# facebookresearch/spdl

Hardware: AMD Instinct MI355X
Metric: images/sec device-resident JPEG→RGB224, 1/2/4/8×MI355X; % HBM roofline (higher is better)
Workload: dtype u8; 1 GPU; configs[1]: synthetic 480x640 q90 4:2:0 baseline JPEG resident in HBM -> RGB 224x224 u8 (scale bicubic decrease + centred pad, rgb24); global_batch=256, per_gpu_batch=256, distinct_images=32, lanes=4, hw_queues=4, entropy_threads=256, entropy_piece_bytes=131072

## Files before the change

spdl_amd/csrc/hj_kernels.hip:

```cpp
#include <hip/hip_fp16.h>
#include <hip/hip_runtime.h>

#include "hj_common.h"
#include "hj_destuff.h"
#include "hj_idct.h"

namespace hj {

__device__ __forceinline__ uint32_t rfl(uint32_t v) { return __builtin_amdgcn_readfirstlane(v); }


struct ParseScratch {
  ImageInfo info;
  uint16_t qt[4][64];
  uint8_t bits[8][17];
  uint8_t vals[8][256];
  int32_t have[8];
  int32_t qhave[4];
  int32_t maxcode[8][18];
  int32_t valoff[8][17];
  int32_t dqt_off[4], dqt_pq[4];
  int32_t dht_off[8], dht_n[8];
  int32_t qtsel[kMaxComp];
  int32_t comp_id[kMaxComp], comp_tq[kMaxComp], order[kMaxComp];
// ... 3787 lines not shown
        out[n++] = ((uint32_t)l[k] << 16) | (uint32_t)k;
      }
    }
    const int32_t dc = (int32_t)(int16_t)(uint16_t)((uint32_t)kDcBias + (uint32_t)l[0] * in.qt[c][0]);
    bdesc[(size_t)dd.coef_off + j] = make_uint2((uint32_t)j * 64u, n | ((uint32_t)dc << 16));
  }
  __syncthreads();
  if (tid == 0) {
    tph[3] = wall_clock64() - t0 - tph[0] - tph[1] - tph[2];
    for (int i = 0; i < 4; i++) in.tphase[i] = tph[i];
    for (int i = 0; i < 4; i++) in.dbg[i] = tdbg[i];
    for (int i = 0; i < 48; i++) in.sdiag[i] = S.sdiag[i];
    in.sync_rounds = S.nscans;
  }
}

hipError_t launch_multiscan(const uint8_t* bytes, uint8_t* clean, const ImageDesc* desc,
                            ImageInfo* infos, uint32_t* ents, uint2* bdesc, int n, hipStream_t st) {
  hipLaunchKernelGGL(multiscan_kernel, dim3(n), dim3(256), 0, st, bytes, clean, desc, infos, ents,
                     bdesc);
  return hipGetLastError();
}


constexpr int kBlkWords = 32;

typedef int16_t __attribute__((may_alias)) hj_i16_alias;

template <int NT>
__device__ __forceinline__ uint32_t slot_byte(uint32_t s) {
  return (s >> 1) * (uint32_t)NT * 4u + ((s & 1u) << 1);
}

template <int NT>
__device__ __forceinline__ void load_dequant(uint32_t (&sq)[kMaxComp][64], const ImageInfo& in,
                                             int tid) {
  for (int k = tid; k < kMaxComp * 64; k += NT)
    sq[k >> 6][k & 63] = slot_byte<NT>(kSlotOrder[k & 63]) | ((uint32_t)in.qt[k >> 6][k & 63] << 16);
}

template <int NT>
__device__ __forceinline__ void list_block(const uint32_t* __restrict__ ents, const uint2 bd,
                                           const int64_t coef_off, const int nblocks,
                                           const uint32_t* sqc, uint32_t* b32) {
#pragma unroll
  for (int w = 0; w < kBlkWords; w++) b32[w * NT] = w == 0 ? (bd.y >> 16) : 0u;
  uint8_t* blk = reinterpret_cast<uint8_t*>(b32);
  uint8_t* dummy = reinterpret_cast<uint8_t*>(b32 + kBlkWords * NT);
  const uint32_t cap = (uint32_t)nblocks * 64u;
  const uint32_t lo = bd.x & 3u, start = bd.x & ~3u;
  uint32_t count = min(bd.y & 0xFFFFu, 63u);
  if (start > cap - 64u) count = 0;
  const uint32_t hi_e = lo + count;
  const uint4* e4 = reinterpret_cast<const uint4*>(ents + (size_t)coef_off * 64 + start);
  const uint32_t n4 = (hi_e + 3u) >> 2;
  for (uint32_t i = 0; i < n4; i += 4) {
    uint4 q[4];
#pragma unroll
    for (int u = 0; u < 4; u++) q[u] = e4[min(i + u, n4 - 1u)];
#pragma unroll
    for (int u = 0; u < 4; u++) {
      const uint32_t w[4] = {q[u].x, q[u].y, q[u].z, q[u].w};
#pragma unroll
      for (int h = 0; h < 4; h++) {
        const uint32_t k = 4u * (i + u) + h;
        const uint32_t qs = sqc[w[h] & 63u];
        uint8_t* dst = k >= lo && k < hi_e ? blk + (qs & 0xFFFFu) : dummy;
        *reinterpret_cast<hj_i16_alias*>(dst) = (int16_t)pk_mul_lo16(w[h] >> 16, qs >> 16);
      }
    }
  }
}

typedef short hj_s16x2 __attribute__((ext_vector_type(2)));
__device__ __forceinline__ int32_t dot2(uint32_t a, uint32_t w, int32_t c) {
  return __builtin_amdgcn_sdot2(__builtin_bit_cast(hj_s16x2, a), __builtin_bit_cast(hj_s16x2, w),
                                c, false);
}
constexpr uint32_t pk16(int lo, int hi) {
  return (uint32_t)(uint16_t)(int16_t)lo | ((uint32_t)(uint16_t)(int16_t)hi << 16);
}
__device__ __forceinline__ uint32_t pack_lo16(uint32_t lo, uint32_t hi) {
  return __builtin_amdgcn_perm(hi, lo, 0x05040100u);
}
__device__ __forceinline__ void sidct8(uint32_t e0, uint32_t e1, uint32_t o0, uint32_t o1,
                                       int32_t bias, int32_t (&a)[4], int32_t (&b)[4]) {
  a[0] = dot2(e1, pk16(kW4, kW6), dot2(e0, pk16(kW4, kW2), bias));
  a[1] = dot2(e1, pk16(-kW4, -kW2), dot2(e0, pk16(kW4, kW6), bias));
  a[2] = dot2(e1, pk16(-kW4, kW2), dot2(e0, pk16(kW4, -kW6), bias));
  a[3] = dot2(e1, pk16(kW4, -kW6), dot2(e0, pk16(kW4, -kW2), bias));
  b[0] = dot2(o1, pk16(kW5, kW7), dot2(o0, pk16(kW1, kW3), 0));
  b[1] = dot2(o1, pk16(-kW1, -kW5), dot2(o0, pk16(kW3, -kW7), 0));
  b[2] = dot2(o1, pk16(kW7, kW3), dot2(o0, pk16(kW5, -kW1), 0));
  b[3] = dot2(o1, pk16(kW3, -kW1), dot2(o0, pk16(kW7, -kW5), 0));
}
template <int NT>
__device__ __forceinline__ uint4 blk_row(const uint32_t* b32, int i) {
  return make_uint4(b32[(4 * i) * NT], b32[(4 * i + 1) * NT], b32[(4 * i + 2) * NT],
                    b32[(4 * i + 3) * NT]);
}
template <int NT>
__device__ __forceinline__ void simple_idct_slots(const uint32_t* b32, int32_t (&px)[64]) {
  uint32_t r[8][8];
#pragma unroll
  for (int i = 0; i < 8; i++) {
    const uint4 q = blk_row<NT>(b32, i);
    int32_t a[4], b[4];
    sidct8(q.x, q.y, q.z, q.w, 1 << 10, a, b);
    const bool dc_only = ((q.x >> 16) | q.y | q.z | q.w) == 0u;
    const uint32_t dc = q.x << 3;
    r[i][0] = dc_only ? dc : (uint32_t)((int32_t)((uint32_t)a[0] + (uint32_t)b[0]) >> 11);
    r[i][7] = dc_only ? dc : (uint32_t)((int32_t)((uint32_t)a[0] - (uint32_t)b[0]) >> 11);
    r[i][1] = dc_only ? dc : (uint32_t)((int32_t)((uint32_t)a[1] + (uint32_t)b[1]) >> 11);
    r[i][6] = dc_only ? dc : (uint32_t)((int32_t)((uint32_t)a[1] - (uint32_t)b[1]) >> 11);
    r[i][2] = dc_only ? dc : (uint32_t)((int32_t)((uint32_t)a[2] + (uint32_t)b[2]) >> 11);
    r[i][5] = dc_only ? dc : (uint32_t)((int32_t)((uint32_t)a[2] - (uint32_t)b[2]) >> 11);
    r[i][3] = dc_only ? dc : (uint32_t)((int32_t)((uint32_t)a[3] + (uint32_t)b[3]) >> 11);
    r[i][4] = dc_only ? dc : (uint32_t)((int32_t)((uint32_t)a[3] - (uint32_t)b[3]) >> 11);
  }
#pragma unroll
  for (int k = 0; k < 8; k++) {
    int32_t a[4], b[4];
    sidct8(pack_lo16(r[0][k], r[2][k]), pack_lo16(r[4][k], r[6][k]), pack_lo16(r[1][k], r[3][k]),
           pack_lo16(r[5][k], r[7][k]), kW4 * ((1 << 19) / kW4), a, b);
    px[k] = clip_u8_opaque((int32_t)((uint32_t)a[0] + (uint32_t)b[0]) >> 20);
    px[8 + k] = clip_u8_opaque((int32_t)((uint32_t)a[1] + (uint32_t)b[1]) >> 20);
    px[16 + k] = clip_u8_opaque((int32_t)((uint32_t)a[2] + (uint32_t)b[2]) >> 20);
    px[24 + k] = clip_u8_opaque((int32_t)((uint32_t)a[3] + (uint32_t)b[3]) >> 20);
    px[32 + k] = clip_u8_opaque((int32_t)((uint32_t)a[3] - (uint32_t)b[3]) >> 20);
    px[40 + k] = clip_u8_opaque((int32_t)((uint32_t)a[2] - (uint32_t)b[2]) >> 20);
    px[48 + k] = clip_u8_opaque((int32_t)((uint32_t)a[1] - (uint32_t)b[1]) >> 20);
    px[56 + k] = clip_u8_opaque((int32_t)((uint32_t)a[0] - (uint32_t)b[0]) >> 20);
  }
}

template <int NT, int IDCT>
__device__ __forceinline__ void idct_block(const uint32_t* b32, int32_t (&px)[64]) {
  if (IDCT == 0) {
    simple_idct_slots<NT>(b32, px);
    return;
  }
  int32_t blk[64];
#pragma unroll
  for (int i = 0; i < 8; i++) {
    const uint4 q = blk_row<NT>(b32, i);
    blk[8 * i + 0] = sext16(q.x);
    blk[8 * i + 2] = sext16(q.x >> 16);
    blk[8 * i + 4] = sext16(q.y);
    blk[8 * i + 6] = sext16(q.y >> 16);
    blk[8 * i + 1] = sext16(q.z);
    blk[8 * i + 3] = sext16(q.z >> 16);
    blk[8 * i + 5] = sext16(q.w);
    blk[8 * i + 7] = sext16(q.w >> 16);
  }
  if (IDCT == 2) {
#pragma unroll
    for (int i = 0; i < 64; i++) px[i] = blk[i] & 255;
  } else {
    islow_block(blk, px);
  }
}

__device__ __forceinline__ void xcd_order(uint32_t& bx, uint32_t& by, uint32_t& bz) {
  const uint32_t n_wg = gridDim.x * gridDim.y * gridDim.z, full = n_wg & ~7u;
  uint32_t lin = bx + gridDim.x * (by + gridDim.y * bz);
  if (lin < full) lin = (lin & 7u) * (full >> 3) + (lin >> 3);
  bx = lin % gridDim.x;
  by = (lin / gridDim.x) % gridDim.y;
  bz = lin / (gridDim.x * gridDim.y);
}

template <int IDCT>
__global__ void __launch_bounds__(kIdctThreads) idct_kernel(const uint32_t* __restrict__ ents,
                                                            const uint2* __restrict__ bdesc,
                                                            const ImageDesc* __restrict__ desc,
                                                            const ImageInfo* __restrict__ infos,
                                                            uint8_t* __restrict__ planes,
                                                            const uint32_t* __restrict__ idct_map,
                                                            const int xcd) {
  __shared__ __attribute__((aligned(16))) uint32_t sblk[kBlkWords + 1][kIdctThreads];
  __shared__ uint32_t sq[kMaxComp][64];
  uint32_t gx = blockIdx.x, gy = blockIdx.y, gz = blockIdx.z;
  if (xcd) xcd_order(gx, gy, gz);
  const bool flat = idct_map != nullptr;
  const int img = flat ? (int)idct_map[gx] : (int)gy;
  const int tile = flat ? (int)gx - desc[img].idct_wg0 : (int)gx;
  const int j = tile * kIdctThreads + threadIdx.x;
  const ImageInfo& in = infos[img];
  if (in.status != kOk || tile * kIdctThreads >= in.nblocks) return;
  load_dequant<kIdctThreads>(sq, in, threadIdx.x);
  __syncthreads();
  if (j >= in.nblocks) return;
  const ImageDesc& dd = desc[img];
  const int bpm = in.bpm;
  const int mcu = j / bpm, b = j - mcu * bpm;
  const int c = in.mcu_comp[b];
  const int mx = mcu % in.mcux, my = mcu / in.mcux;
  int bx, by;
  if (in.ncomp == 1) {
    bx = mx;
    by = my;
  } else {
    bx = mx * in.comp_h[c] + in.mcu_dx[b];
    by = my * in.comp_v[c] + in.mcu_dy[b];
  }
  uint32_t* b32 = &sblk[0][threadIdx.x];
  list_block<kIdctThreads>(ents, bdesc[(size_t)dd.coef_off + j], dd.coef_off, in.nblocks, sq[c],
                           b32);
  int32_t px[64];
  idct_block<kIdctThreads, IDCT>(b32, px);
  const int stride = dd.plane_stride[c];
  uint8_t* dst = planes + dd.plane_off[c] + (size_t)by * 8 * stride + bx * 8;
#pragma unroll
  for (int r = 0; r < 8; r++) {
    uint2 v;
    v.x = (uint32_t)px[8 * r] | ((uint32_t)px[8 * r + 1] << 8) | ((uint32_t)px[8 * r + 2] << 16) |
          ((uint32_t)px[8 * r + 3] << 24);
    v.y = (uint32_t)px[8 * r + 4] | ((uint32_t)px[8 * r + 5] << 8) |
          ((uint32_t)px[8 * r + 6] << 16) | ((uint32_t)px[8 * r + 7] << 24);
    *reinterpret_cast<uint2*>(dst + (size_t)r * stride) = v;
  }
}


constexpr int32_t kFix1402 = 91881, kFix1772 = 116130, kFix0714 = 46802, kFix0344 = 22553;

__device__ __forceinline__ void ycc_rgb(int y, int cb, int cr, int* rgb) {
  const int32_t x_cb = cb - 128, x_cr = cr - 128;
  const int32_t cr_r = (kFix1402 * x_cr + 32768) >> 16;
  const int32_t cb_b = (kFix1772 * x_cb + 32768) >> 16;
  const int32_t g = ((-kFix0344 * x_cb + 32768) + (-kFix0714 * x_cr)) >> 16;
  rgb[0] = clip_u8(y + cr_r);
  rgb[1] = clip_u8(y + g);
  rgb[2] = clip_u8(y + cb_b);
}

__device__ __forceinline__ uint16_t to_f16_bits(float f, int dtype) {
  if (dtype == 1) return __half_as_ushort(__float2half_rn(f));
  uint32_t x = __float_as_uint(f);
  if ((x & 0x7FFFFFFFu) > 0x7F800000u) return (uint16_t)((x >> 16) | 0x40u);
  x += 0x7FFFu + ((x >> 16) & 1u);
  return (uint16_t)(x >> 16);
}

__device__ __forceinline__ void store_rgb(void* out, int64_t base, int fmt, int dtype, int ow,
                                          int oh, int x, int y, const int* rgb,
                                          const BatchParams& p) {
  const bool planar = fmt == 0 || fmt == 1;
  const bool swap = fmt == 1 || fmt == 3;
  const int64_t pl = (int64_t)ow * oh;
#pragma unroll
  for (int ch = 0; ch < 3; ch++) {
    const int v = rgb[swap ? 2 - ch : ch];
    const int64_t oi = base + (planar ? ch * pl + (int64_t)y * ow + x : ((int64_t)y * ow + x) * 3 + ch);
    if (dtype == 0) {
      static_cast<uint8_t*>(out)[oi] = (uint8_t)v;
    } else {
      float f = __fdiv_rn((float)v, 255.0f);
      f = __fsub_rn(f, p.mean[ch]);
      f = __fdiv_rn(f, p.std[ch]);
      static_cast<uint16_t*>(out)[oi] = to_f16_bits(f, dtype);
    }
  }
}

__global__ void __launch_bounds__(256) csc_kernel(const uint8_t* __restrict__ planes,
                                                  const ImageDesc* __restrict__ desc,
                                                  const ImageInfo* __restrict__ infos,
                                                  void* __restrict__ out, const BatchParams p,
                                                  int32_t* __restrict__ host_status) {
  const int img = blockIdx.y;
  const ImageInfo& in = infos[img];
  if (host_status && blockIdx.x == 0 && threadIdx.x == 0) host_status[img] = in.status;
  if (in.status != kOk) return;
  const ImageDesc& dd = desc[img];
  const int W = in.width, H = in.height;
  const int64_t npx = (int64_t)W * H;
  for (int64_t i = (int64_t)blockIdx.x * blockDim.x + threadIdx.x; i < npx;
       i += (int64_t)gridDim.x * blockDim.x) {
    const int y = (int)(i / W), x = (int)(i - (int64_t)y * W);
    const int lx = x * in.comp_h[0] / in.hmax, ly = y * in.comp_v[0] / in.vmax;
    const int yv = planes[dd.plane_off[0] + (int64_t)ly * dd.plane_stride[0] + lx];
    int rgb[3];
    if (in.ncomp == 1) {
      rgb[0] = rgb[1] = rgb[2] = yv;
    } else {
      const int cx1 = x * in.comp_h[1] / in.hmax, cy1 = y * in.comp_v[1] / in.vmax;
      const int cx2 = x * in.comp_h[2] / in.hmax, cy2 = y * in.comp_v[2] / in.vmax;
      const int cb = planes[dd.plane_off[1] + (int64_t)cy1 * dd.plane_stride[1] + cx1];
      const int cr = planes[dd.plane_off[2] + (int64_t)cy2 * dd.plane_stride[2] + cx2];
      if (in.color == kColorRgb) {
        rgb[0] = yv;
        rgb[1] = cb;
        rgb[2] = cr;
      } else {
        ycc_rgb(yv, cb, cr, rgb);
      }
    }
    store_rgb(out, dd.out_off, p.pix_fmt, p.dtype, W, H, x, y, rgb, p);
  }
}


typedef short hj_short2 __attribute__((ext_vector_type(2)));
typedef uint32_t hj_u32x4a __attribute__((ext_vector_type(4), aligned(4)));

template <int NW>
__device__ __forceinline__ void load_words(const uint8_t* p, uint32_t (&w)[NW]) {
  static_assert(NW % 4 == 0, "whole 16-byte loads");
#pragma unroll
  for (int i = 0; i < NW; i += 4) {
    const hj_u32x4a v = *reinterpret_cast<const hj_u32x4a*>(p + 4 * i);
    w[i] = v.x;
    w[i + 1] = v.y;
    w[i + 2] = v.z;
    w[i + 3] = v.w;
  }
}

template <int NQ, int NW>
__device__ __forceinline__ int32_t hdot(const uint32_t (&w)[NW], uint32_t sh, const uint32_t* wp) {
  int32_t h = 0;
#pragma unroll
  for (int i = 0; i < NQ; i++) {
    const uint32_t u = __builtin_amdgcn_alignbyte(w[i + 1], w[i], sh);
    const uint32_t lo = __builtin_amdgcn_perm(0u, u, 0x0C010C00u);
    const uint32_t hi = __builtin_amdgcn_perm(0u, u, 0x0C030C02u);
    h = __builtin_amdgcn_sdot2(__builtin_bit_cast(hj_short2, lo),
                               __builtin_bit_cast(hj_short2, wp[2 * i]), h, false);
    h = __builtin_amdgcn_sdot2(__builtin_bit_cast(hj_short2, hi),
                               __builtin_bit_cast(hj_short2, wp[2 * i + 1]), h, false);
  }
  return h;
}

__device__ __forceinline__ int16_t h15(int32_t h) {
  return (int16_t)min(h >> 7, (1 << 15) - 1);
}

template <int NQ>
__device__ __forceinline__ void hpass_cols(const uint8_t* plane, int stride, int ph, const int32_t* pos,
                           const int16_t* coef, int cstride, int c0, int ncols, int r0, int r1,
                           int16_t* lds, int cst, int tid, int nthreads, int rst = 1) {
  constexpr int NW = (NQ + 1 + 3) / 4 * 4;
  for (int c = tid; c < ncols; c += nthreads) {
    const int x = c0 + c;
    const int p = pos[x];
    const uint32_t sh = (uint32_t)(p & 3);
    uint32_t wp[2 * NQ];
    const uint2* cp = reinterpret_cast<const uint2*>(coef + (int64_t)x * cstride);
#pragma unroll
    for (int k = 0; k < NQ; k++) {
      const uint2 t = cp[k];
      wp[2 * k] = t.x;
      wp[2 * k + 1] = t.y;
    }
    const uint8_t* base = plane + (p & ~3);
    int16_t* out = lds + c * cst;
    constexpr int G = NW <= 4 ? 12 : (NW <= 8 ? 4 : 1);
    for (int r = r0; r < r1; r += G) {
      uint32_t w[G][NW];
#pragma unroll
      for (int g = 0; g < G; g++)
        if (r + g < r1) load_words<NW>(base + (int64_t)min(r + g, ph - 1) * stride, w[g]);
#pragma unroll
      for (int g = 0; g < G; g++)
        if (r + g < r1) out[(r + g - r0) * rst] = h15(hdot<NQ>(w[g], sh, wp));
    }
  }
}

__device__ __forceinline__ void hpass_cols_long(const uint8_t* plane, int stride, int ph, const int32_t* pos,
                                const int16_t* coef, int cstride, int taps, int c0, int ncols,
                                int r0, int r1, int16_t* lds, int cst, int tid, int nthreads,
                                int rst = 1) {
  for (int c = tid; c < ncols; c += nthreads) {
    const int x = c0 + c;
    const int p = pos[x];
    const int16_t* cf = coef + (int64_t)x * cstride;
    for (int r = r0; r < r1; r++) {
      const uint8_t* row = plane + (int64_t)min(r, ph - 1) * stride + p;
      int32_t v = 0;
      for (int t = 0; t < taps; t++) v += (int32_t)row[t] * cf[t];
      lds[c * cst + (r - r0) * rst] = h15(v);
    }
  }
}

__device__ __forceinline__ void hpass(const uint8_t* plane, int stride, int ph, const int32_t* pos,
                      const int16_t* coef, int cstride, int taps, int c0, int ncols, int r0, int r1,
                      int16_t* lds, int cst, int tid, int nthreads, int rst = 1) {
  const int nq = (taps + 3) >> 2;
#define HJ_HP(N) \
  hpass_cols<N>(plane, stride, ph, pos, coef, cstride, c0, ncols, r0, r1, lds, cst, tid, nthreads, \
                rst)
  if (nq <= 1) HJ_HP(1);
  else if (nq <= 2) HJ_HP(2);
  else if (nq <= 3) HJ_HP(3);
  else if (nq <= 4) HJ_HP(4);
  else if (nq <= 6) HJ_HP(6);
  else if (nq <= 8) HJ_HP(8);
  else if (nq <= 12) HJ_HP(12);
  else if (nq <= 16) HJ_HP(16);
  else hpass_cols_long(plane, stride, ph, pos, coef, cstride, taps, c0, ncols, r0, r1, lds, cst, tid,
                       nthreads, rst);
#undef HJ_HP
}

__device__ __forceinline__ int32_t vdot_pairs(const uint32_t* col, int p, const uint32_t* f,
                                              int np) {
  const uint32_t* c = col + (p >> 1);
  const uint32_t sh = (uint32_t)(p & 1) * 16u;
  int32_t acc = 0;
  uint32_t w0 = c[0];
  for (int i = 0; i < np; i += 2) {
    const uint32_t w1 = c[i + 1], w2 = c[i + 2];
    const uint2 ff = *reinterpret_cast<const uint2*>(f + i);
    acc = __builtin_amdgcn_sdot2(__builtin_bit_cast(hj_short2, __builtin_amdgcn_alignbit(w1, w0, sh)),
                                 __builtin_bit_cast(hj_short2, ff.x), acc, false);
    acc = __builtin_amdgcn_sdot2(__builtin_bit_cast(hj_short2, __builtin_amdgcn_alignbit(w2, w1, sh)),
                                 __builtin_bit_cast(hj_short2, ff.y), acc, false);
    w0 = w2;
  }
  return acc;
}

__device__ __forceinline__ void vpair(const uint32_t* col, int p, int& a, int& b) {
  const uint32_t* c = col + (p >> 1);
  const uint32_t w = __builtin_amdgcn_alignbit(c[1], c[0], (uint32_t)(p & 1) * 16u);
  a = (int32_t)(int16_t)(w & 0xFFFFu);
  b = (int32_t)w >> 16;
}

__device__ __forceinline__ int clip_i8(int v) { return v < 0 ? 0 : (v > 255 ? 255 : v); }

__device__ __forceinline__ int tab_off(int32_t inc, int c) {
  return ((clip_i8(c) * inc) >> 16) - (inc >> 9);
}

__device__ __forceinline__ void full_rgb(const BatchParams& p, int Y, int U, int V, int* rgb) {
  Y -= p.y_offset;
  Y *= p.y_coeff;
  Y += 1 << 21;
  int R = (int)((uint32_t)Y + (uint32_t)V * (uint32_t)p.v2r);
  int G = (int)((uint32_t)Y + (uint32_t)V * (uint32_t)p.v2g + (uint32_t)U * (uint32_t)p.u2g);
  int B = (int)((uint32_t)Y + (uint32_t)U * (uint32_t)p.u2b);
  if ((R | G | B) & 0xC0000000) {
    auto c30 = [](int a) { return (a & ~((1 << 30) - 1)) ? ((~a) >> 31) & ((1 << 30) - 1) : a; };
    R = c30(R);
    G = c30(G);
    B = c30(B);
  }
  rgb[0] = R >> 22;
  rgb[1] = G >> 22;
  rgb[2] = B >> 22;
}

__global__ void __launch_bounds__(256) hscale_kernel(const uint8_t* __restrict__ planes,
                                                     const ImageDesc* __restrict__ desc,
                                                     const ImageInfo* __restrict__ infos,
                                                     const int32_t* __restrict__ pool,
                                                     const uint32_t* __restrict__ hs_map,
                                                     int16_t* __restrict__ hbuf) {
  const int img = (int)hs_map[blockIdx.x];
  const ImageInfo& in = infos[img];
  if (in.status != kOk) return;
  const ImageDesc& dd = desc[img];
  const SwsDesc& s = dd.sws;
  const int32_t* T = pool + dd.wt_off;
  const int tl = (s.pre_rl + kHsRows - 1) / kHsRows;
  const int tc = s.gbr ? tl : (s.gray ? 0 : (s.pre_rc + kHsRows - 1) / kHsRows);
  int t = (int)blockIdx.x - dd.hs_wg0;
  int c = 0;
  if (t >= tl) {
    t -= tl;
    c = 1 + t / tc;
    t %= tc;
  }
  const bool lumaf = c == 0 || s.gbr;
  const int rows = lumaf ? s.pre_rl : s.pre_rc;
  const int w = lumaf ? s.sw : s.chr_w;
  const int r0 = t * kHsRows, r1 = min(r0 + kHsRows, rows);
  const int64_t pbase = c == 0 ? 0 : (int64_t)s.pre_rl * s.sw + (c == 1 ? 0 : (int64_t)rows * w);
  const uint8_t* plane = planes + dd.plane_off[c];
  const int stride = dd.plane_stride[c], ph = in.comp_hpx[c];
  const int32_t* pos = T + s.off[lumaf ? kHlPos : kHcPos];
  const int16_t* coef = reinterpret_cast<const int16_t*>(T + s.off[lumaf ? kHlCoef : kHcCoef]);
  const int cstride = lumaf ? s.hl_size : s.hc_size, taps = lumaf ? s.hl_taps : s.hc_taps;
  int16_t* dst = hbuf + dd.hbuf_off + pbase + (int64_t)r0 * w;
  if (taps <= 64) {
    hpass(plane, stride, ph, pos, coef, cstride, taps, 0, w, r0, r1, dst, 1, threadIdx.x,
          blockDim.x, w);
    return;
  }
  const int nch = (taps + 63) / 64;
  for (int x = threadIdx.x; x < w; x += blockDim.x) {
    const int p0 = pos[x];
    const uint32_t sh = (uint32_t)(p0 & 3);
    const uint8_t* base = plane + (p0 & ~3);
    int32_t acc[kHsRows];
#pragma unroll
    for (int g = 0; g < kHsRows; g++) acc[g] = 0;
    for (int k = 0; k < nch; k++) {
      uint32_t wp[32];
      const uint2* cp = reinterpret_cast<const uint2*>(coef + (int64_t)x * cstride + 64 * k);
#pragma unroll
      for (int q = 0; q < 16; q++) {
        const bool in_row = 64 * k + 4 * q < taps;
        const uint2 t = in_row ? cp[q] : make_uint2(0u, 0u);
        wp[2 * q] = t.x;
        wp[2 * q + 1] = t.y;
      }
#pragma unroll
      for (int g = 0; g < kHsRows; g++) {
        if (r0 + g >= r1) break;
        uint32_t wv[20];
        load_words<20>(base + (int64_t)min(r0 + g, ph - 1) * stride + 64 * k, wv);
        acc[g] += hdot<16>(wv, sh, wp);
      }
    }
#pragma unroll
    for (int g = 0; g < kHsRows; g++)
      if (r0 + g < r1) dst[(int64_t)g * w + x] = h15(acc[g]);
  }
}

__global__ void __launch_bounds__(256) sws_kernel(const uint8_t* __restrict__ planes,
                                                  const ImageDesc* __restrict__ desc,
                                                  const ImageInfo* __restrict__ infos,
                                                  const int32_t* __restrict__ pool,
                                                  void* __restrict__ out, const BatchParams p,
                                                  int32_t* __restrict__ host_status,
                                                  const int16_t* __restrict__ hbuf,
                                                  const uint32_t* __restrict__ sws_map) {
  extern __shared__ __attribute__((aligned(16))) int16_t sws_lds[];
  const bool flat = sws_map != nullptr;
  uint32_t bx = blockIdx.x, by = blockIdx.y, bz = blockIdx.z;
  if (p.xcd_order & 1) xcd_order(bx, by, bz);
  const int img = flat ? (int)sws_map[bx] : (int)bz, tid = threadIdx.x, nt = blockDim.x;
  const ImageDesc& dd = desc[img];
  const int t = flat ? (int)bx - dd.sws_wg0 : (int)(bx * dd.sws_chunks + by);
  const int band = flat ? t / dd.sws_chunks : (int)bx;
  const int chunk = flat ? t - band * dd.sws_chunks : (int)by;
  const ImageInfo& in = infos[img];
  if (host_status && t == 0 && tid == 0) host_status[img] = in.status;
  if (in.status != kOk) return;
  const SwsDesc& s = dd.sws;
  const int yo0 = band * s.rb, xo0 = chunk * s.col_chunk;
  if (yo0 >= dd.oh || xo0 >= dd.ow) return;
  const int yo1 = min(yo0 + s.rb, dd.oh), xo1 = min(xo0 + s.col_chunk, dd.ow);
  const int th = yo1 - yo0, tw = xo1 - xo0;
  const int ys0 = max(yo0 - dd.dy, 0), ys1 = min(yo1 - dd.dy, s.sh);
  const int xs0 = max(xo0 - dd.dx, 0), xs1 = min(xo1 - dd.dx, s.sw);
  const bool content = ys0 < ys1 && xs0 < xs1;
  const bool planar = p.pix_fmt == 0 || p.pix_fmt == 1;
  const bool swap = p.pix_fmt == 1 || p.pix_fmt == 3;
  const bool u8 = p.dtype == 0;
  const int64_t pl = (int64_t)dd.ow * dd.oh;
  const int32_t* T = pool + dd.wt_off;
  const int32_t* vl_pos = T + s.off[kVlPos];
  const int32_t* vc_pos = T + s.off[kVcPos];
  int lr0 = 0, lr1 = 0, cr0 = 0, cr1 = 0, cx0 = 0, ncc = 0;
  const int ncl = content ? xs1 - xs0 : 0;
  if (content) {
    lr0 = vl_pos[ys0];
    lr1 = vl_pos[ys1 - 1] + s.vl_taps;
    if (!s.gray) {
      cr0 = vc_pos[ys0];
      cr1 = vc_pos[ys1 - 1] + s.vc_taps;
      cx0 = s.full ? xs0 : xs0 >> 1;
      ncc = (s.full ? xs1 - 1 : (xs1 - 1) >> 1) + 1 - cx0;
    }
  }
  const int lst = sws_col_stride(lr1 - lr0), cst = sws_col_stride(cr1 - cr0);
  int16_t* hl = sws_lds;
  int16_t* hu = hl + ncl * lst;
  int16_t* hv = hu + (s.gbr ? ncl * lst : s.gray ? 0 : ncc * cst);
  const int hrow_end = (int)((hv + (s.gbr ? ncl * lst : s.gray ? 0 : ncc * cst)) - sws_lds);
  uint8_t* tile = reinterpret_cast<uint8_t*>(sws_lds) + ((2 * hrow_end + 15) & ~15);
  const int vrw = 4 + (s.vl_size + s.vc_size) / 2;
  uint32_t* vt = reinterpret_cast<uint32_t*>(tile + ((s.rb * s.col_chunk * 3 + 15) & ~15));
  if (content) {
    const int32_t* vmode = T + s.off[kVmode];
    const uint32_t* vlw = reinterpret_cast<const uint32_t*>(T + s.off[kVlCoef]);
    const uint32_t* vcw = reinterpret_cast<const uint32_t*>(T + s.off[kVcCoef]);
    const int nl = s.vl_size / 2, nc = s.vc_size / 2;
    for (int i = tid; i < (ys1 - ys0) * vrw; i += nt) {
      const int r = i / vrw, w = i - r * vrw, ys = ys0 + r;
      uint32_t v = 0;
      if (w == 0) v = (uint32_t)vmode[ys];
      else if (w == 1) v = (uint32_t)(vl_pos[ys] - lr0);
      else if (w == 2) v = s.gray ? 0u : (uint32_t)(vc_pos[ys] - cr0);
      else if (w >= 4 && w < 4 + nl) v = vlw[(int64_t)ys * nl + (w - 4)];
      else if (w >= 4 + nl) v = vcw[(int64_t)ys * nc + (w - 4 - nl)];
      vt[i] = v;
    }
  }
  auto put = [&](int xo, int yo, const int* rgb) {
    const int c0v = swap ? rgb[2] : rgb[0], c2v = swap ? rgb[0] : rgb[2];
    const int cv[3] = {c0v, rgb[1], c2v};
    if (u8) {
#pragma unroll
      for (int ch = 0; ch < 3; ch++) {
        const int v = cv[ch];
        const int ti = planar ? (ch * th + (yo - yo0)) * tw + (xo - xo0)
                              : ((yo - yo0) * tw + (xo - xo0)) * 3 + ch;
        tile[ti] = (uint8_t)v;
      }
      return;
    }
#pragma unroll
    for (int ch = 0; ch < 3; ch++) {
      const int v = cv[ch];
      const int64_t oi =
          dd.out_off + (planar ? ch * pl + (int64_t)yo * dd.ow + xo : ((int64_t)yo * dd.ow + xo) * 3 + ch);
      float f = __fdiv_rn((float)v, 255.0f);
      f = __fsub_rn(f, p.mean[ch]);
      f = __fdiv_rn(f, p.std[ch]);
      static_cast<uint16_t*>(out)[oi] = to_f16_bits(f, p.dtype);
    }
  };
  {
    const int npx = th * tw;
    const int zero[3] = {0, 0, 0};
    for (int i = tid; i < npx; i += nt) {
      const int yo = yo0 + i / tw, xo = xo0 + i % tw;
      const int ys = yo - dd.dy, xs = xo - dd.dx;
      if (ys < 0 || ys >= s.sh || xs < 0 || xs >= s.sw) put(xo, yo, zero);
    }
  }
  if (content && s.pre) {
    const int16_t* hb = hbuf + dd.hbuf_off;
    const int wl = s.sw, wc = s.gbr ? s.sw : s.chr_w;
    const int64_t cbase = (int64_t)s.pre_rl * wl;
    auto stage = [&](const int16_t* src, int w, int rows, int c0, int ncols, int r0, int r1,
                     int16_t* dst, int cst_) {
      const int nr = r1 - r0, ne = ncols * nr;
      for (int i0 = tid; i0 < ne; i0 += 4 * nt) {
        int16_t v[4];
#pragma unroll
        for (int u = 0; u < 4; u++) {
          const int i = min(i0 + u * nt, ne - 1);
          const int r = i / ncols, c = i - r * ncols;
          v[u] = src[(int64_t)min(r0 + r, rows - 1) * w + c0 + c];
        }
#pragma unroll
        for (int u = 0; u < 4; u++) {
          const int i = i0 + u * nt;
          if (i < ne) {
            const int r = i / ncols, c = i - r * ncols;
            dst[c * cst_ + r] = v[u];
          }
        }
      }
    };
    stage(hb, wl, s.pre_rl, xs0, ncl, lr0, lr1, hl, lst);
    if (s.gbr) {
      stage(hb + cbase, wl, s.pre_rl, xs0, ncl, lr0, lr1, hu, lst);
      stage(hb + 2 * cbase, wl, s.pre_rl, xs0, ncl, lr0, lr1, hv, lst);
    } else if (!s.gray) {
      const int64_t cpl = (int64_t)s.pre_rc * wc;
      stage(hb + cbase, wc, s.pre_rc, cx0, ncc, cr0, cr1, hu, cst);
      stage(hb + cbase + cpl, wc, s.pre_rc, cx0, ncc, cr0, cr1, hv, cst);
    }
  } else if (content && s.gbr) {
    const int third = nt / 3, c = min(tid / third, 2), t3 = tid - c * third;
    if (tid < 3 * third)
      hpass(planes + dd.plane_off[c], dd.plane_stride[c], in.comp_hpx[c], T + s.off[kHlPos],
            reinterpret_cast<const int16_t*>(T + s.off[kHlCoef]), s.hl_size, s.hl_taps, xs0, ncl,
            lr0, lr1, c == 0 ? hl : c == 1 ? hu : hv, lst, t3, third);
  } else if (content && !(p.debug_mask & 0x100)) {
    hpass(planes + dd.plane_off[0], dd.plane_stride[0], in.comp_hpx[0], T + s.off[kHlPos],
          reinterpret_cast<const int16_t*>(T + s.off[kHlCoef]), s.hl_size, s.hl_taps, xs0, ncl,
          lr0, lr1, hl, lst, tid, nt);
    if (!s.gray) {
      const int half = nt >> 1, t2 = tid < half ? tid : tid - half;
      const int c = tid < half ? 1 : 2;
      hpass(planes + dd.plane_off[c], dd.plane_stride[c], in.comp_hpx[c], T + s.off[kHcPos],
            reinterpret_cast<const int16_t*>(T + s.off[kHcCoef]), s.hc_size, s.hc_taps, cx0, ncc,
            cr0, cr1, c == 1 ? hu : hv, cst, t2, half);
    }
  }
  __syncthreads();
  if (content && !(p.debug_mask & 0x200)) {
    const int npl = s.vl_size / 2, npc = s.vc_size / 2;
    for (int cl = tid; cl < ncl; cl += nt) {
      const int xs = xs0 + cl;
      const int cc = (s.full ? xs : xs >> 1) - cx0;
      const uint32_t* lcol = reinterpret_cast<const uint32_t*>(hl + cl * lst);
      const uint32_t* ucol = reinterpret_cast<const uint32_t*>(hu + cc * cst);
      const uint32_t* vcol = reinterpret_cast<const uint32_t*>(hv + cc * cst);
      for (int ys = ys0; ys < ys1; ys++) {
        const uint32_t* row = vt + (ys - ys0) * vrw;
        const uint4 hdr = *reinterpret_cast<const uint4*>(row);
        const int m = (int)hdr.x;
        const int mode = m & 15, ya = (m >> 4) & 8191, ua = (m >> 17) & 8191;
        const uint32_t* lf = row + 4;
        const uint32_t* cf = lf + npl;
        const int lp = (int)hdr.y, cp = (int)hdr.z;
        int rgb[3];
        int Y, U = 0, V = 0;
        if (s.gbr) {
          const uint32_t* cols[3] = {lcol, lcol + (hu - hl) / 2, lcol + (hv - hl) / 2};
#pragma unroll
          for (int c = 0; c < 3; c++) {
            int v;
            if (mode == kSwsX) {
              v = ((1 << 18) + vdot_pairs(cols[c], lp, lf, npl)) >> 19;
            } else {
              int a, b;
              vpair(cols[c], lp, a, b);
              v = mode == kSwsTwo ? (a * (4096 - ya) + b * ya) >> 19 : (a + 64) >> 7;
            }
            rgb[c] = clip_i8(v);
          }
        } else if (s.full) {
          if (mode == kSwsTwo) {
            int a, b;
            vpair(lcol, lp, a, b);
            Y = (a * (4096 - ya) + b * ya) >> 10;
          } else if (mode == kSwsOne) {
            int a, b;
            vpair(lcol, lp, a, b);
            Y = a * 4;
          } else {
            Y = ((1 << 9) + vdot_pairs(lcol, lp, lf, npl)) >> 10;
          }
          if (!s.gray) {
            if (mode == kSwsX) {
              U = ((1 << 9) - (128 << 19) + vdot_pairs(ucol, cp, cf, npc)) >> 10;
              V = ((1 << 9) - (128 << 19) + vdot_pairs(vcol, cp, cf, npc)) >> 10;
            } else {
              int u0, u1, v0, v1;
              vpair(ucol, cp, u0, u1);
              vpair(vcol, cp, v0, v1);
              if (!ua) {
                u1 = u0;
                v1 = v0;
              }
              U = (u0 * (4096 - ua) + u1 * ua - (128 << 19)) >> 10;
              V = (v0 * (4096 - ua) + v1 * ua - (128 << 19)) >> 10;
            }
          }
          full_rgb(p, Y, U, V, rgb);
        } else {
          if (mode == kSwsX) {
            Y = ((1 << 18) + vdot_pairs(lcol, lp, lf, npl)) >> 19;
            U = ((1 << 18) + vdot_pairs(ucol, cp, cf, npc)) >> 19;
            V = ((1 << 18) + vdot_pairs(vcol, cp, cf, npc)) >> 19;
          } else {
            int y0, y1, u0, u1, v0, v1;
            vpair(lcol, lp, y0, y1);
            vpair(ucol, cp, u0, u1);
            vpair(vcol, cp, v0, v1);
            if (mode == kSwsTwo) {
              Y = (y0 * (4096 - ya) + y1 * ya) >> 19;
              U = (u0 * (4096 - ua) + u1 * ua) >> 19;
              V = (v0 * (4096 - ua) + v1 * ua) >> 19;
            } else {
              if (!ua) {
                u1 = u0;
                v1 = v0;
              }
              Y = (y0 + 64) >> 7;
              U = (u0 * (4096 - ua) + u1 * ua + (128 << 11)) >> 19;
              V = (v0 * (4096 - ua) + v1 * ua + (128 << 11)) >> 19;
            }
          }
          rgb[0] = clip_i8(Y + tab_off(p.crv, V));
          rgb[1] = clip_i8(Y + tab_off(p.cgu, U) + tab_off(p.cgv, V));
          rgb[2] = clip_i8(Y + tab_off(p.cbu, U));
        }
        put(xs + dd.dx, ys + dd.dy, rgb);
      }
    }
  }
  if (!u8 || (p.debug_mask & 0x400)) return;
  __syncthreads();
  const int nplane = planar ? 3 : 1;
  const int run = planar ? th * tw : th * tw * 3;
  for (int pc = 0; pc < nplane; pc++) {
    const uint8_t* src = tile + pc * run;
    uint8_t* dst = static_cast<uint8_t*>(out) + dd.out_off + pc * pl +
                   (planar ? (int64_t)yo0 * dd.ow + xo0 : ((int64_t)yo0 * dd.ow + xo0) * 3);
    if (tw == dd.ow && ((uintptr_t)dst & 15) == 0 && (run & 15) == 0) {
      for (int i = tid; i < run / 16; i += nt)
        reinterpret_cast<uint4*>(dst)[i] = reinterpret_cast<const uint4*>(src)[i];
    } else {
      const int rowb = planar ? tw : tw * 3;
      const int64_t ostride = planar ? dd.ow : (int64_t)dd.ow * 3;
      for (int i = tid; i < run; i += nt) {
        const int r = i / rowb, k = i - r * rowb;
        dst[r * ostride + k] = src[i];
      }
    }
  }
}

__device__ __forceinline__ void yuv_stage(const int16_t* __restrict__ src, int w, int rows, int c0,
                                          int ncols, int r0, int r1, int16_t* dst, int cst,
                                          int tid, int nt) {
  const int nr = r1 - r0, ne = ncols * nr;
  for (int i0 = tid; i0 < ne; i0 += 4 * nt) {
    int16_t v[4];
#pragma unroll
    for (int u = 0; u < 4; u++) {
      const int i = min(i0 + u * nt, ne - 1);
      const int r = i / ncols, c = i - r * ncols;
      v[u] = src[(int64_t)min(r0 + r, rows - 1) * w + c0 + c];
    }
#pragma unroll
    for (int u = 0; u < 4; u++) {
      const int i = i0 + u * nt;
      if (i < ne) {
        const int r = i / ncols, c = i - r * ncols;
        dst[c * cst + r] = v[u];
      }
    }
  }
}

__global__ void __launch_bounds__(256) yuv_planes_kernel(const uint8_t* __restrict__ planes,
                                                         const ImageDesc* __restrict__ desc,
                                                         const ImageInfo* __restrict__ infos,
                                                         const int32_t* __restrict__ pool,
                                                         uint8_t* __restrict__ out,
                                                         int32_t* __restrict__ host_status,
                                                         const int16_t* __restrict__ hbuf,
                                                         const uint32_t* __restrict__ sws_map) {
  extern __shared__ __attribute__((aligned(16))) int16_t yuv_lds[];
  const int img = (int)sws_map[blockIdx.x], tid = threadIdx.x, nt = blockDim.x;
  const ImageDesc& dd = desc[img];
  int t = (int)blockIdx.x - dd.sws_wg0;
  const ImageInfo& in = infos[img];
  if (host_status && t == 0 && tid == 0) host_status[img] = in.status;
  if (in.status != kOk) return;
  const SwsDesc& s = dd.sws;
  const int cw = (dd.ow + (1 << s.hsub) - 1) >> s.hsub, ch = (dd.oh + (1 << s.vsub) - 1) >> s.vsub;
  const int ltiles = ((dd.oh + s.rb - 1) / s.rb) * ((dd.ow + s.col_chunk - 1) / s.col_chunk);
  int c = 0;
  if (t >= ltiles) {
    const int ctiles = ((ch + s.rb - 1) / s.rb) * ((cw + s.col_chunk - 1) / s.col_chunk);
    t -= ltiles;
    c = 1 + t / ctiles;
    t -= (c - 1) * ctiles;
    if (s.gray || c > 2) return;
  }
  const bool luma = c == 0;
  const int W = luma ? dd.ow : cw, H = luma ? dd.oh : ch;
  const int psw = luma ? s.sw : s.chr_w, psh = luma ? s.sh : s.chr_h;
  const int pdx = luma ? dd.dx : dd.dx >> s.hsub, pdy = luma ? dd.dy : dd.dy >> s.vsub;
  const int padv = luma ? (s.gray ? 16 : 0) : 128;
  const int chunks = (W + s.col_chunk - 1) / s.col_chunk;
  const int band = t / chunks, chunk = t - band * chunks;
  const int yo0 = band * s.rb, xo0 = chunk * s.col_chunk;
  if (yo0 >= H || xo0 >= W) return;
  const int yo1 = min(yo0 + s.rb, H), xo1 = min(xo0 + s.col_chunk, W);
  const int th = yo1 - yo0, tw = xo1 - xo0;
  const int ys0 = max(yo0 - pdy, 0), ys1 = min(yo1 - pdy, psh);
  const int xs0 = max(xo0 - pdx, 0), xs1 = min(xo1 - pdx, psw);
  const bool content = ys0 < ys1 && xs0 < xs1;
  const int ncl = content ? xs1 - xs0 : 0;
  const int32_t* T = pool + dd.wt_off;
  const int32_t* vpos = T + s.off[luma ? kVlPos : kVcPos];
  const uint32_t* vco = reinterpret_cast<const uint32_t*>(T + s.off[luma ? kVlCoef : kVcCoef]);
  const int vnp = (luma ? s.vl_size : s.vc_size) / 2, vtaps = luma ? s.vl_taps : s.vc_taps;
  int r0 = 0, r1 = 0;
  if (content) {
    r0 = vpos[ys0];
    r1 = vpos[ys1 - 1] + vtaps;
  }
  const int cst = sws_col_stride(r1 - r0);
  int16_t* hcol = yuv_lds;
  uint8_t* tile = reinterpret_cast<uint8_t*>(yuv_lds) + ((2 * ncl * cst + 15) & ~15);
  const int64_t pbase = dd.out_off + (luma ? 0 : (int64_t)dd.ow * dd.oh + (int64_t)(c - 1) * cw * ch);
  uint8_t* dst = out + pbase + (int64_t)yo0 * W + xo0;
  const bool whole = tw == W;
  const int nrun = whole ? 1 : th, runlen = whole ? th * W : tw;
  const int pitch = (tw + 30) & ~15;
  const uint32_t g0 = (uint32_t)(uintptr_t)dst;
  auto tpos = [&](int r, int k) {
    return whole ? (int)(g0 & 15u) + r * W + k : r * pitch + (int)((g0 + (uint32_t)(r * W)) & 15u) + k;
  };
  for (int i = tid; i < th * tw; i += nt) {
    const int r = i / tw, k = i - r * tw;
    const int ys = yo0 + r - pdy, xs = xo0 + k - pdx;
    if (ys < 0 || ys >= psh || xs < 0 || xs >= psw) tile[tpos(r, k)] = (uint8_t)padv;
  }
  if (content && s.pre) {
    const int64_t poff = luma ? 0 : (int64_t)s.pre_rl * s.sw + (int64_t)(c - 1) * s.pre_rc * s.chr_w;
    yuv_stage(hbuf + dd.hbuf_off + poff, psw, luma ? s.pre_rl : s.pre_rc, xs0, ncl, r0, r1, hcol,
              cst, tid, nt);
  } else if (content) {
    hpass(planes + dd.plane_off[c], dd.plane_stride[c], in.comp_hpx[c],
          T + s.off[luma ? kHlPos : kHcPos],
          reinterpret_cast<const int16_t*>(T + s.off[luma ? kHlCoef : kHcCoef]),
          luma ? s.hl_size : s.hc_size, luma ? s.hl_taps : s.hc_taps, xs0, ncl, r0, r1, hcol, cst,
          tid, nt);
  }
  __syncthreads();
  if (content) {
    for (int cl = tid; cl < ncl; cl += nt) {
      const uint32_t* col = reinterpret_cast<const uint32_t*>(hcol + cl * cst);
      const int k = xs0 + cl + pdx - xo0;
      for (int ys = ys0; ys < ys1; ys++) {
        const int v = ((1 << 18) + vdot_pairs(col, vpos[ys] - r0, vco + (int64_t)ys * vnp, vnp)) >> 19;
        tile[tpos(ys + pdy - yo0, k)] = (uint8_t)clip_i8(v);
      }
    }
  }
  __syncthreads();
  const int items = 30 + runlen / 16 + 1;
  for (int i = tid; i < nrun * items; i += nt) {
    const int r = i / items, j = i - r * items;
    uint8_t* g = dst + (int64_t)r * W;
    const uint8_t* l = tile + tpos(r, 0);
    const int head = min(runlen, (int)((16u - ((uint32_t)(uintptr_t)g & 15u)) & 15u));
    const int nvec = (runlen - head) >> 4, tail = runlen - head - 16 * nvec;
    if (j < 15) {
      if (j < head) g[j] = l[j];
    } else if (j < 30) {
      const int o = head + 16 * nvec + (j - 15);
      if (j - 15 < tail) g[o] = l[o];
    } else if (j - 30 < nvec) {
      const int o = head + 16 * (j - 30);
      *reinterpret_cast<uint4*>(g + o) = *reinterpret_cast<const uint4*>(l + o);
    }
  }
}

constexpr int kRgbPx = 8;

template <int N>
__device__ __forceinline__ void rgbu_load(const uint8_t* p, uint32_t (&w)[N]) {
  if constexpr (N == 1) {
    w[0] = *reinterpret_cast<const uint32_t*>(p);
  } else if constexpr (N == 2) {
    const uint2 v = *reinterpret_cast<const uint2*>(p);
    w[0] = v.x, w[1] = v.y;
  } else {
    static_assert(N == 4, "rgbu_load: 1, 2 or 4 words");
    const uint4 v = *reinterpret_cast<const uint4*>(p);
    w[0] = v.x, w[1] = v.y, w[2] = v.z, w[3] = v.w;
  }
}

template <int N>
__device__ __forceinline__ void rgbu_store(uint8_t* p, const uint32_t* w) {
  if constexpr (N == 2) {
    *reinterpret_cast<uint2*>(p) = make_uint2(w[0], w[1]);
  } else {
    static_assert(N == 4, "rgbu_store: 2 or 4 words");
    *reinterpret_cast<uint4*>(p) = make_uint4(w[0], w[1], w[2], w[3]);
  }
}

template <int PX>
__device__ __forceinline__ void rgbu_group(const uint32_t (&yw)[PX / 4], const uint32_t (&uw)[PX / 8],
                                           const uint32_t (&vw)[PX / 8], uint8_t* __restrict__ base,
                                           const int64_t pl, const int w, const int y, const int x0,
                                           const int npx, const BatchParams& p, const bool planar,
                                           const bool swap) {
  constexpr int SW = PX / 4;
  uint32_t c0[PX], c1[PX], c2[PX];
#pragma unroll
  for (int i = 0; i < PX; i++) {
    const int Y = (int)((yw[i >> 2] >> (8 * (i & 3))) & 0xFFu);
    const int U = (int)((uw[i >> 3] >> (8 * ((i >> 1) & 3))) & 0xFFu);
    const int V = (int)((vw[i >> 3] >> (8 * ((i >> 1) & 3))) & 0xFFu);
    const int r = clip_i8(Y + tab_off(p.crv, V));
    const int gg = clip_i8(Y + tab_off(p.cgu, U) + tab_off(p.cgv, V));
    const int b = clip_i8(Y + tab_off(p.cbu, U));
    c0[i] = (uint32_t)(swap ? b : r);
    c1[i] = (uint32_t)gg;
    c2[i] = (uint32_t)(swap ? r : b);
  }
  if (!planar) {
    uint8_t* o = base + ((int64_t)y * w + x0) * 3;
    if (npx == PX && ((uintptr_t)o & (4u * SW - 1u)) == 0u) {
      uint32_t wv[3 * PX / 4];
#pragma unroll
      for (int k = 0; k < 3 * PX / 4; k++) {
        uint32_t v = 0;
#pragma unroll
        for (int j = 0; j < 4; j++) {
          const int q = 4 * k + j, i = q / 3, c = q % 3;
          v |= (c == 0 ? c0[i] : c == 1 ? c1[i] : c2[i]) << (8 * j);
// ... 367 lines not shown
```

Measured before the change: 571,500 images/sec.

## Use dot4 horizontal taps, paired-chroma vertical pass, and rectangle pad fill

The horizontal scaler pass switches from sdot2 on widened pixel pairs to udot4/sdot4 on packed bytes, splitting each 16-bit tap into low and high byte halves and precomputing a bias correction. The vertical/colour pass for 4:2:0 input now has each lane handle two luma pixels that share one chroma column, so U/V interpolation and colour-table lookups run once per pixel pair and work is spread over waves by row and chunk. Padding is zeroed only over the border rectangles, using word stores, instead of testing every output pixel. This cuts ALU work and redundant chroma computation, at the cost of more complex indexing and a risk of rounding or edge differences.

New measurement: 591,800 images/sec (median of 6 runs). +3.6%, better.

```diff
diff --git a/spdl_amd/csrc/hj_kernels.hip b/spdl_amd/csrc/hj_kernels.hip
--- a/spdl_amd/csrc/hj_kernels.hip
+++ b/spdl_amd/csrc/hj_kernels.hip
@@ -4113,6 +4113,16 @@
 }
 
 
+#ifndef HJ_SWS_PADRECT
+#define HJ_SWS_PADRECT 1
+#endif
+#ifndef HJ_SWS_PAIRS
+#define HJ_SWS_PAIRS 1
+#endif
+#ifndef HJ_SWS_DOT4
+#define HJ_SWS_DOT4 1
+#endif
+
 typedef short hj_short2 __attribute__((ext_vector_type(2)));
 typedef uint32_t hj_u32x4a __attribute__((ext_vector_type(4), aligned(4)));
 
@@ -4143,6 +4153,26 @@
                                __builtin_bit_cast(hj_short2, wp[2 * i + 1]), h, false);
   }
   return h;
+}
+
+template <int NQ, int NW>
+__device__ __forceinline__ int32_t hdot4(const uint32_t (&w)[NW], uint32_t sh, const uint32_t* wp,
+                                         int32_t k0) {
+  uint32_t a = 0;
+  int32_t b = k0;
+#pragma unroll
+  for (int i = 0; i < NQ; i++) {
+    const uint32_t u = __builtin_amdgcn_alignbyte(w[i + 1], w[i], sh);
+    a = __builtin_amdgcn_udot4(u, wp[2 * i], a, false);
+    b = __builtin_amdgcn_sdot4((int32_t)(u ^ 0x80808080u), (int32_t)wp[2 * i + 1], b, false);
+  }
+  return (int32_t)(a + ((uint32_t)b << 8));
+}
+
+__device__ __forceinline__ int32_t split_taps(uint2 t, uint32_t& lo, uint32_t& hi, int32_t sum) {
+  lo = __builtin_amdgcn_perm(t.y, t.x, 0x06040200u);
+  hi = __builtin_amdgcn_perm(t.y, t.x, 0x07050301u);
+  return __builtin_amdgcn_sdot4((int32_t)hi, 0x01010101, sum, false);
 }
 
 __device__ __forceinline__ int16_t h15(int32_t h) {
@@ -4160,12 +4190,19 @@
     const uint32_t sh = (uint32_t)(p & 3);
     uint32_t wp[2 * NQ];
     const uint2* cp = reinterpret_cast<const uint2*>(coef + (int64_t)x * cstride);
+#if HJ_SWS_DOT4
+    int32_t k0 = 0;
+#pragma unroll
+    for (int k = 0; k < NQ; k++) k0 = split_taps(cp[k], wp[2 * k], wp[2 * k + 1], k0);
+    k0 <<= 7;
+#else
 #pragma unroll
     for (int k = 0; k < NQ; k++) {
       const uint2 t = cp[k];
       wp[2 * k] = t.x;
       wp[2 * k + 1] = t.y;
     }
+#endif
     const uint8_t* base = plane + (p & ~3);
     int16_t* out = lds + c * cst;
     constexpr int G = NW <= 4 ? 12 : (NW <= 8 ? 4 : 1);
@@ -4176,7 +4213,11 @@
         if (r + g < r1) load_words<NW>(base + (int64_t)min(r + g, ph - 1) * stride, w[g]);
 #pragma unroll
       for (int g = 0; g < G; g++)
+#if HJ_SWS_DOT4
+        if (r + g < r1) out[(r + g - r0) * rst] = h15(hdot4<NQ>(w[g], sh, wp, k0));
+#else
         if (r + g < r1) out[(r + g - r0) * rst] = h15(hdot<NQ>(w[g], sh, wp));
+#endif
     }
   }
 }
@@ -4234,6 +4275,32 @@
     w0 = w2;
   }
   return acc;
+}
+
+__device__ __forceinline__ void vdot_pairs2(const uint32_t* col0, const uint32_t* col1, int p,
+                                            const uint32_t* f, int np, int32_t& acc0,
+                                            int32_t& acc1) {
+  const uint32_t* c0 = col0 + (p >> 1);
+  const uint32_t* c1 = col1 + (p >> 1);
+  const uint32_t sh = (uint32_t)(p & 1) * 16u;
+  int32_t a0 = 0, a1 = 0;
+  uint32_t x0 = c0[0], y0 = c1[0];
+  for (int i = 0; i < np; i += 2) {
+    const uint32_t x1 = c0[i + 1], x2 = c0[i + 2], y1 = c1[i + 1], y2 = c1[i + 2];
+    const uint2 ff = *reinterpret_cast<const uint2*>(f + i);
+    a0 = __builtin_amdgcn_sdot2(__builtin_bit_cast(hj_short2, __builtin_amdgcn_alignbit(x1, x0, sh)),
+                                __builtin_bit_cast(hj_short2, ff.x), a0, false);
+    a1 = __builtin_amdgcn_sdot2(__builtin_bit_cast(hj_short2, __builtin_amdgcn_alignbit(y1, y0, sh)),
+                                __builtin_bit_cast(hj_short2, ff.x), a1, false);
+    a0 = __builtin_amdgcn_sdot2(__builtin_bit_cast(hj_short2, __builtin_amdgcn_alignbit(x2, x1, sh)),
+                                __builtin_bit_cast(hj_short2, ff.y), a0, false);
+    a1 = __builtin_amdgcn_sdot2(__builtin_bit_cast(hj_short2, __builtin_amdgcn_alignbit(y2, y1, sh)),
+                                __builtin_bit_cast(hj_short2, ff.y), a1, false);
+    x0 = x2;
+    y0 = y2;
+  }
+  acc0 = a0;
+  acc1 = a1;
 }
 
 __device__ __forceinline__ void vpair(const uint32_t* col, int p, int& a, int& b) {
@@ -4407,9 +4474,8 @@
       vt[i] = v;
     }
   }
-  auto put = [&](int xo, int yo, const int* rgb) {
-    const int c0v = swap ? rgb[2] : rgb[0], c2v = swap ? rgb[0] : rgb[2];
-    const int cv[3] = {c0v, rgb[1], c2v};
+  auto putc = [&](int xo, int yo, int c0v, int c1v, int c2v) {
+    const int cv[3] = {c0v, c1v, c2v};
     if (u8) {
 #pragma unroll
       for (int ch = 0; ch < 3; ch++) {
@@ -4431,6 +4497,49 @@
       static_cast<uint16_t*>(out)[oi] = to_f16_bits(f, p.dtype);
     }
   };
+  auto put = [&](int xo, int yo, const int* rgb) {
+    putc(xo, yo, swap ? rgb[2] : rgb[0], rgb[1], swap ? rgb[0] : rgb[2]);
+  };
+#if HJ_SWS_PADRECT
+  {
+    const int cy0 = content ? ys0 + dd.dy : yo1, cy1 = content ? ys1 + dd.dy : yo1;
+    const int cxa = xs0 + dd.dx, cxb = xs1 + dd.dx;
+    if (cy0 > yo0 || cy1 < yo1 || cxa > xo0 || cxb < xo1) {
+      const int lane = tid & 63, nw = nt >> 6;
+      const int wave = __builtin_amdgcn_readfirstlane(tid >> 6);
+      auto zrun = [&](int off, int n, int t, int nth) {
+        const int head = min(n, -off & 3), words = (n - head) >> 2;
+        const int tail = n - head - 4 * words;
+        uint8_t* q = tile + off + head;
+        if (t < head) tile[off + t] = 0;
+        for (int i = t; i < words; i += nth) reinterpret_cast<uint32_t*>(q)[i] = 0u;
+        if (t < tail) q[4 * words + t] = 0;
+      };
+      auto fill = [&](int ya, int yb, int xa, int xb) {
+        if (ya >= yb || xa >= xb) return;
+        if (!u8) {
+          for (int yo = ya + wave; yo < yb; yo += nw)
+            for (int xo = xa + lane; xo < xb; xo += 64) putc(xo, yo, 0, 0, 0);
+          return;
+        }
+        const int bpp = planar ? 1 : 3, np_ = planar ? 3 : 1;
+        const int ps = th * tw;
+        if (xb - xa == tw) {
+          for (int pc = 0; pc < np_; pc++)
+            zrun((pc * ps + (ya - yo0) * tw) * bpp, (yb - ya) * tw * bpp, tid, nt);
+          return;
+        }
+        for (int yo = ya + wave; yo < yb; yo += nw)
+          for (int pc = 0; pc < np_; pc++)
+            zrun((pc * ps + (yo - yo0) * tw + (xa - xo0)) * bpp, (xb - xa) * bpp, lane, 64);
+      };
+      fill(yo0, cy0, xo0, xo1);
+      fill(cy1, yo1, xo0, xo1);
+      fill(cy0, cy1, xo0, cxa);
+      fill(cy0, cy1, cxb, xo1);
+    }
+  }
+#else
   {
     const int npx = th * tw;
     const int zero[3] = {0, 0, 0};
@@ -4440,6 +4549,7 @@
       if (ys < 0 || ys >= s.sh || xs < 0 || xs >= s.sw) put(xo, yo, zero);
     }
   }
+#endif
   if (content && s.pre) {
     const int16_t* hb = hbuf + dd.hbuf_off;
     const int wl = s.sw, wc = s.gbr ? s.sw : s.chr_w;
@@ -4493,7 +4603,82 @@
     }
   }
   __syncthreads();
-  if (content && !(p.debug_mask & 0x200)) {
+#if HJ_SWS_PAIRS
+  const bool pairs = !s.full && !s.gbr && !s.gray;
+#else
+  const bool pairs = false;
+#endif
+  if (content && pairs && !(p.debug_mask & 0x200)) {
+    const int npl = s.vl_size / 2, npc = s.vc_size / 2;
+    const int lane = tid & 63, nw = nt >> 6;
+    const int wave = __builtin_amdgcn_readfirstlane(tid >> 6);
+    const int nch = (ncc + 63) >> 6, nrows = ys1 - ys0;
+    int r = 0, chk = wave;
+    while (chk >= nch) {
+      chk -= nch;
+      r++;
+    }
+    while (r < nrows) {
+      const uint32_t* row = vt + r * vrw;
+      const uint4 hdr = *reinterpret_cast<const uint4*>(row);
+      const int m = (int)hdr.x;
+      const int lp = (int)hdr.y, cp = (int)hdr.z;
+      const int mode = m & 15, ya = (m >> 4) & 8191, ua = (m >> 17) & 8191;
+      const uint32_t* lf = row + 4;
+      const uint32_t* cf = lf + npl;
+      const int cc = chk * 64 + lane;
+      if (cc < ncc) {
+        const int xe = 2 * (cx0 + cc) - xs0;
+        const bool h0 = xe >= 0, h1 = xe + 1 < ncl;
+        const uint32_t* l0 = reinterpret_cast<const uint32_t*>(hl + max(xe, 0) * lst);
+        const uint32_t* l1 = reinterpret_cast<const uint32_t*>(hl + min(xe + 1, ncl - 1) * lst);
+        const uint32_t* ucol = reinterpret_cast<const uint32_t*>(hu + cc * cst);
+        const uint32_t* vcol = reinterpret_cast<const uint32_t*>(hv + cc * cst);
+        int Y0, Y1, U, V;
+        if (mode == kSwsX) {
+          int32_t a0, a1;
+          vdot_pairs2(l0, l1, lp, lf, npl, a0, a1);
+          Y0 = ((1 << 18) + a0) >> 19;
+          Y1 = ((1 << 18) + a1) >> 19;
+          vdot_pairs2(ucol, vcol, cp, cf, npc, a0, a1);
+          U = ((1 << 18) + a0) >> 19;
+          V = ((1 << 18) + a1) >> 19;
+        } else {
+          int y00, y01, y10, y11, u0, u1, v0, v1;
+          vpair(l0, lp, y00, y01);
+          vpair(l1, lp, y10, y11);
+          vpair(ucol, cp, u0, u1);
+          vpair(vcol, cp, v0, v1);
+          if (mode == kSwsTwo) {
+            Y0 = (y00 * (4096 - ya) + y01 * ya) >> 19;
+            Y1 = (y10 * (4096 - ya) + y11 * ya) >> 19;
+            U = (u0 * (4096 - ua) + u1 * ua) >> 19;
+            V = (v0 * (4096 - ua) + v1 * ua) >> 19;
+          } else {
+            if (!ua) {
+              u1 = u0;
+              v1 = v0;
+            }
+            Y0 = (y00 + 64) >> 7;
+            Y1 = (y10 + 64) >> 7;
+            U = (u0 * (4096 - ua) + u1 * ua + (128 << 11)) >> 19;
+            V = (v0 * (4096 - ua) + v1 * ua + (128 << 11)) >> 19;
+          }
+        }
+        const int tr = tab_off(p.crv, V), tb = tab_off(p.cbu, U);
+        const int t0 = swap ? tb : tr, t2 = swap ? tr : tb;
+        const int t1 = tab_off(p.cgu, U) + tab_off(p.cgv, V);
+        const int yo = ys0 + r + dd.dy, xo = xs0 + xe + dd.dx;
+        if (h0) putc(xo, yo, clip_i8(Y0 + t0), clip_i8(Y0 + t1), clip_i8(Y0 + t2));
+        if (h1) putc(xo + 1, yo, clip_i8(Y1 + t0), clip_i8(Y1 + t1), clip_i8(Y1 + t2));
+      }
+      chk += nw;
+      while (chk >= nch) {
+        chk -= nch;
+        r++;
+      }
+    }
+  } else if (content && !(p.debug_mask & 0x200)) {
     const int npl = s.vl_size / 2, npc = s.vc_size / 2;
     for (int cl = tid; cl < ncl; cl += nt) {
       const int xs = xs0 + cl;
```
